# thorfdbg/libjpeg

Measured on AMD Instinct MI355X. Metric: decoded Mpixels/s, 8K 4:2:0 baseline (fused IDCT+upsample+YCbCr kernel, coefficients resident in HBM), higher is better.
Workload: dtype int32 (int16 coefficients in, u8 pixels out); 1 GPU; 64 x 7680x4320 4:2:0 Q85 DRI=8 baseline frames per GPU per step (BASELINE configs[2] frame shape, device-resident coefficient planes; 2 distinct pictures per rank repeated over the 64 frames: 6075 MiB in + 6075 MiB out per launch, far beyond the 256 MiB Infinity Cache); frames_per_gpu=64, kernel=fused420p_kernel, settle_launches=64, fast_arith=1, parallelism=image-sharded x1, no data-path collective

## Files before the change

### libjpeg_amd/csrc/kernels.hip

```cpp

#include <hip/hip_runtime.h>
#include <type_traits>
#include <stdint.h>
#include <stdlib.h>

#include "kernels.hpp"

namespace mij {

typedef unsigned u32x4 __attribute__((ext_vector_type(4)));
typedef unsigned u32x2 __attribute__((ext_vector_type(2)));
typedef u32x2 u32x2_any __attribute__((aligned(1)));
typedef u32x4 u32x4_any __attribute__((aligned(1)));
typedef int i32x4 __attribute__((ext_vector_type(4)));

template <bool FAST>
__device__ __forceinline__ int mulc(int a, int c)
{
  if (FAST) return __mul24(a, c);
  return (int)((unsigned)a * (unsigned)c);
}
__device__ __forceinline__ int addw(int a, int b) { return (int)((unsigned)a + (unsigned)b); }
__device__ __forceinline__ int subw(int a, int b) { return (int)((unsigned)a - (unsigned)b); }
__device__ __forceinline__ int shlw(int a, int n) { return (int)((unsigned)a << n); }
// ... 795 lines not shown
struct LdsPairHalf {
  short *cp;
  __device__ __forceinline__ LdsPairHalf(unsigned *cpair, int comp) : cp(reinterpret_cast<short *>(cpair) + comp) {}
  __device__ __forceinline__ void one(int at, int v) const { cp[2 * at] = (short)v; }
  __device__ __forceinline__ void row8(int at, const int *v) const
  {
    short *dst = cp + 2 * at;
#pragma unroll
    for (int x = 0; x < 8; x++) dst[2 * x] = (short)v[x];
  }
};
struct LdsPlane32 {
  int *cp;
  __device__ __forceinline__ LdsPlane32(int *plane) : cp(plane) {}
  __device__ __forceinline__ void one(int at, int v) const { cp[at] = v; }
  __device__ __forceinline__ void row8(int at, const int *v) const
  {
    i32x4 *dst = reinterpret_cast<i32x4 *>(cp + at);
    dst[0] = i32x4{v[0], v[1], v[2], v[3]};
    dst[1] = i32x4{v[4], v[5], v[6], v[7]};
  }
};

constexpr int F420P_MINW = 4;
constexpr int F420_FAST_MINW = 2;
constexpr int F420_12_MINW = 2;

struct NoAfterFetch { __device__ __forceinline__ void operator()() const {} };
template <bool FAST, bool QDEV = false, bool PK = false, class AfterFetch = NoAfterFetch>
__device__ __forceinline__ void f420_chroma_to_lds(const Fused420Args &a, const TileCtx &t, int (*cplane)[F420_CROWS * F420_CPITCH],
                                                   AfterFetch after_fetch = AfterFetch())
{
  const int16_t *__restrict__ coef = t.coef;
  u32x4 *stage = t.stage;
  const int lane = t.lane, wave = t.wave, tx = t.tx, ty = t.ty, frame = t.frame;
  const int comp = wave >> 1;
  const int16_t *__restrict__ plane = coef + (comp ? a.off_cr : a.off_cb);
  const int gx0 = tx * 8 - 1, gy0 = ty * 8 - 1;
  const int base = (wave & 1) * 64;
  const bool inside = gx0 >= 0 && gy0 >= 0 && gx0 + F420_CGRID <= a.bw_c && gy0 + F420_CGRID <= a.bh_c;
  u32x4 rows[8];
  const int idx0 = base + (lane >> 3);
  const char *pbase = reinterpret_cast<const char *>(plane) + (lane & 7) * 16;
  if (inside) {
    const unsigned off0 = (unsigned)((gy0 * a.bw_c + gx0) * 128), rowb = (unsigned)a.bw_c * 128u;
    fetch_blocks(rows, stage, lane, [&](int m) -> const u32x4 * {
      const unsigned i = (unsigned)min(idx0 + 8 * m, F420_CGRID * F420_CGRID - 1);
      const unsigned y = (i * 205u) >> 11, x = i - y * F420_CGRID;
      return reinterpret_cast<const u32x4 *>(pbase + (off0 + y * rowb + x * 128u));
    });
  } else {
    fetch_blocks(rows, stage, lane, [&](int m) -> const u32x4 * {
      const int i = min(idx0 + 8 * m, F420_CGRID * F420_CGRID - 1);
      const int y = (i * 205) >> 11, x = i - y * F420_CGRID;
      const int gx = min(max(gx0 + x, 0), a.bw_c - 1), gy = min(max(gy0 + y, 0), a.bh_c - 1);
      return reinterpret_cast<const u32x4 *>(pbase + (unsigned)((gy * a.bw_c + gx) * 128));
    });
  }
  after_fetch();
  if constexpr (!std::is_same<AfterFetch, NoAfterFetch>::value) __builtin_amdgcn_sched_barrier(0);
  const int idx = base + lane;
  const int cby = idx / F420_CGRID, cbx = idx - cby * F420_CGRID;
  const int gx = gx0 + cbx, gy = gy0 + cby;
  if (idx < F420_CGRID * F420_CGRID && gx >= 0 && gy >= 0 && gx < a.bw_c && gy < a.bh_c) {
    int v[64];
    const int *q = frame_deltas<QDEV>(a, frame, 1 + comp);
    if (FAST) dequant_idct_sparse<PK>(rows, q, v);
    else dequant_idct<false>(rows, q, v, 128 << 7);
    int *cp = cplane[comp];
#pragma unroll
    for (int r = 0; r < 8; r++) {
      const int pr = 8 * cby + r - 7;
      if (pr >= 0 && pr < F420_CROWS) {
        if (cbx == 0) {
          cp[pr * F420_CPITCH + 3] = v[r * 8 + 7];
        } else if (cbx == F420_CGRID - 1) {
          cp[pr * F420_CPITCH + 68] = v[r * 8 + 0];
        } else {
          i32x4 *dst = reinterpret_cast<i32x4 *>(cp + pr * F420_CPITCH + 8 * cbx - 4);
          dst[0] = i32x4{v[r * 8 + 0], v[r * 8 + 1], v[r * 8 + 2], v[r * 8 + 3]};
          dst[1] = i32x4{v[r * 8 + 4], v[r * 8 + 5], v[r * 8 + 6], v[r * 8 + 7]};
        }
      }
    }
  }
}

__device__ __forceinline__ void f420_chroma_edges(const Fused420Args &a, int (*cplane)[F420_CROWS * F420_CPITCH], int tid, int tx, int ty)
{
  const int last_col = a.cw - 1 - tx * 64;
  const int last_row = a.ch - 1 - ty * 64;
  const bool edge = (tx == 0) | (ty == 0) | (last_col < 64) | (last_row < 64);
  if (edge) {
    if (tid < 2 * F420_CROWS) {
      int *p = cplane[tid / F420_CROWS] + (tid % F420_CROWS) * F420_CPITCH;
      if (tx == 0) p[3] = p[4];
      if (last_col < 64) {
        const int v = p[last_col + 4];
        for (int pc = last_col + 5; pc <= 68; pc++) p[pc] = v;
      }
    }
    __syncthreads();
    if (tid < 2 * F420_CROWS) {
      int *p = cplane[tid / F420_CROWS] + 3 + (tid % F420_CROWS);
      if (ty == 0) p[0] = p[F420_CPITCH];
      if (last_row < 64) {
        const int v = p[(last_row + 1) * F420_CPITCH];
        for (int pr = last_row + 2; pr < F420_CROWS; pr++) p[pr * F420_CPITCH] = v;
      }
    }
    __syncthreads();
  }
}

constexpr int F422_CROWS = 128;
template <bool QDEV, bool PK16, class STORE>
__device__ __forceinline__ void f422_chroma_to_lds(const Fused420Args &a, const TileCtx &t, const STORE cp)
{
  const int lane = t.lane, wave = t.wave;
  const int comp = wave >> 1;
  const int16_t *__restrict__ plane = t.coef + (comp ? a.off_cr : a.off_cb);
  const int gx0 = t.tx * 8, gy0 = t.ty * 16 + (wave & 1) * 8;
  const char *pbase = reinterpret_cast<const char *>(plane) + (lane & 7) * 16;
  u32x4 rows[8];
  {
    const int xx = min(gx0 + (lane >> 3), a.bw_c - 1);
    fetch_blocks(rows, t.stage, lane, [&](int m) -> const u32x4 * {
      const int yy = min(gy0 + m, a.bh_c - 1);
      return reinterpret_cast<const u32x4 *>(pbase + (unsigned)((yy * a.bw_c + xx) * 128));
    });
    const int cbx = lane & 7, cby = lane >> 3;
    if (gx0 + cbx < a.bw_c && gy0 + cby < a.bh_c) {
      int v[64];
      dequant_idct_sparse<PK16>(rows, frame_deltas<QDEV>(a, t.frame, 1 + comp), v);
#pragma unroll
      for (int r = 0; r < 8; r++) cp.row8((8 * ((wave & 1) * 8 + cby) + r) * F420_CPITCH + 8 * cbx + 4, v + r * 8);
    }
  }
  {
    fetch_blocks16(rows, t.stage, lane, [&](int m) -> const u32x4 * {
      const int n = (lane >> 3) + 8 * m;
      const int xx = min(max((n & 1) ? gx0 + 8 : gx0 - 1, 0), a.bw_c - 1), yy = min(gy0 + (n >> 1), a.bh_c - 1);
      return reinterpret_cast<const u32x4 *>(pbase + (unsigned)((yy * a.bw_c + xx) * 128));
    });
    const int side = lane & 1, cby = lane >> 1, gx = side ? gx0 + 8 : gx0 - 1;
    if (lane < 16 && gx >= 0 && gx < a.bw_c && gy0 + cby < a.bh_c) {
      int col[8];
      dequant_idct_column(rows, frame_deltas<QDEV>(a, t.frame, 1 + comp), side == 0, col);
#pragma unroll
      for (int r = 0; r < 8; r++) cp.one((8 * ((wave & 1) * 8 + cby) + r) * F420_CPITCH + (side ? 68 : 3), col[r]);
    }
  }
}

template <int PLANES, class T>
__device__ __forceinline__ void f422_chroma_edges(const Fused420Args &a, T *lines, int tid, int tx)
{
  const int last_col = a.cw - 1 - tx * 64;
  if ((tx == 0) | (last_col < 64)) {
    if (tid < PLANES * F422_CROWS) {
      T *p = lines + tid * F420_CPITCH;
      if (tx == 0) p[3] = p[4];
      if (last_col < 64) {
        const T v = p[last_col + 4];
        for (int pc = last_col + 5; pc <= 68; pc++) p[pc] = v;
      }
    }
    __syncthreads();
  }
}

template <bool FAST, int MINW, bool QDEV, int P = 8, bool N12 = false, bool RAGGED = false>
__global__ __launch_bounds__(F420_THREADS, MINW) void fused420_kernel(Fused420Args a)
{
  static_assert(P == 8 || (P == 12 && FAST), "12-bit frames: FAST flavour only (the host checks the ranges)");
  static_assert(!RAGGED || (QDEV && P == 8), "ragged launches: 8 bit, per-frame tables");
  __shared__ __attribute__((aligned(16))) int cplane[2][F420_CROWS * F420_CPITCH];
  __shared__ __attribute__((aligned(16))) u32x4 stage_all[4][128];

  const TileCtx t = RAGGED ? tile_enter_ragged(a, stage_all) : tile_enter<P == 8 ? MIJ_TILE_ORDER : 1>(a, stage_all);
  if (t.padding) return;

  u32x4 yraw[8];
  auto luma_loads = [&]() { load_tile_blocks(yraw, t, t.coef + a.off_y, a.bw_y, a.bh_y); };
  constexpr bool PREFETCH = P == 8;
  if (PREFETCH) f420_chroma_to_lds<FAST, QDEV, !QDEV && P == 8>(a, t, cplane, luma_loads);
  else f420_chroma_to_lds<FAST, QDEV, !QDEV && P == 8>(a, t, cplane);
  __syncthreads();
  f420_chroma_edges(a, cplane, t.tid, t.tx, t.ty);

  u32x4 rows[8];
  if (!PREFETCH) luma_loads();
  transpose_blocks(rows, t.stage, t.lane, yraw);
  const BlockOut o = block_out<P == 12 ? 6 : 3>(a, t);
  if (o.outside) return;
  int yv[64];
  if (FAST) dequant_idct_sparse<!QDEV && P == 8, P == 8>(rows, frame_deltas<QDEV>(a, t.frame, 0), yv, 0, P == 8 ? LUMA_FOLD_R2 : 2048);
  else dequant_idct<false>(rows, frame_deltas<QDEV>(a, t.frame, 0), yv, 128 << 7);

  const int *cb_base = cplane[0] + (4 * o.by) * F420_CPITCH + 4 * o.bx;
  const int *cr_base = cplane[1] + (4 * o.by) * F420_CPITCH + 4 * o.bx;

  int cbT[6], cbC[6], cbB[6], crT[6], crC[6], crB[6];
  load6(cb_base, cbT); load6(cb_base + F420_CPITCH, cbC);
  load6(cr_base, crT); load6(cr_base + F420_CPITCH, crC);

#pragma unroll
  for (int m = 0; m < 4; m++) {
    load6(cb_base + (m + 2) * F420_CPITCH, cbB);
    load6(cr_base + (m + 2) * F420_CPITCH, crB);
#pragma unroll
    for (int half = 0; half < 2; half++) {
      const int l = 2 * m + half;
      int vb[6], vr[6];
#pragma unroll
      for (int j = 0; j < 6; j++) {
        const int rnd = ((j & 1) ^ half) ? 1 : 2;
        vb[j] = tap13(half ? cbB[j] : cbT[j], cbC[j], rnd);
        vr[j] = tap13(half ? crB[j] : crT[j], crC[j], rnd);
      }
      int ub[8], ur[8];
      hfilter8(vb, ub);
      hfilter8(vr, ur);
      if (l < o.nln) {
        if (FAST && P == 12) {
          int rr[8], gg[8], bb[8];
#pragma unroll
          for (int x = 0; x < 8; x++) colour12<N12>(yv[l * 8 + x], ub[x], ur[x], rr[x], gg[x], bb[x]);
          store_rgb12_line<F420_12_TEMPORAL>(o.out_frame + o.line_off(l, a), rr, gg, bb, o.fast_store, o.npx);
        } else if (FAST) {
          int rr[8], gg[8], bb[8];
#pragma unroll
          for (int x = 0; x < 8; x++) {
            const int yk = luma13(yv[l * 8 + x]);
            rr[x] = mad24(ur[x], L_CR_R, yk);
            gg[x] = mad24(ur[x], -L_CR_G, mad24(ub[x], -L_CB_G, yk));
            bb[x] = mad24(ub[x], L_CB_B, yk);
          }
          store_rgb8_line<STORE24_3X8>(o.out_frame, o.line_off(l, a), rr, gg, bb, o.fast_store, o.npx);
        } else {
          uint8_t *dst = o.out_frame + o.line_off(l, a);
          unsigned px[24];
#pragma unroll
          for (int x = 0; x < 8; x++) {
            int r, g, b;
            ycc_to_rgb<false>(yv[l * 8 + x], ub[x], ur[x], r, g, b);
            px[3 * x] = r; px[3 * x + 1] = g; px[3 * x + 2] = b;
          }
          if (o.fast_store) {
            unsigned w[6];
#pragma unroll
            for (int i = 0; i < 6; i++) w[i] = px[4 * i] | (px[4 * i + 1] << 8) | (px[4 * i + 2] << 16) | (px[4 * i + 3] << 24);
            store24_3x8(dst, w);
          } else {
#pragma unroll
            for (int x = 0; x < 8; x++)
              if (x < o.npx) {
                dst[3 * x] = (uint8_t)px[3 * x]; dst[3 * x + 1] = (uint8_t)px[3 * x + 1]; dst[3 * x + 2] = (uint8_t)px[3 * x + 2];
              }
          }
        }
      }
    }
#pragma unroll
    for (int j = 0; j < 6; j++) { cbT[j] = cbC[j]; cbC[j] = cbB[j]; crT[j] = crC[j]; crC[j] = crB[j]; }
  }
}

typedef short s16x2 __attribute__((ext_vector_type(2)));

__device__ __forceinline__ unsigned tap13_pk(unsigned a, unsigned b, short r)
{
  const s16x2 va = __builtin_bit_cast(s16x2, a), vb = __builtin_bit_cast(s16x2, b);
  const s16x2 t = (va + vb * (short)3 + r) >> (short)2;
  return __builtin_bit_cast(unsigned, t);
}
__device__ __forceinline__ unsigned centre3_pk(unsigned b, short r)
{
  unsigned d;
  asm("v_pk_mad_u16 %0, %1, 3, %2 op_sel_hi:[1,0,0]" : "=v"(d) : "v"(b), "n"(r));
  return d;
}
__device__ __forceinline__ unsigned tap_sum_pk(unsigned a, unsigned w)
{
  const s16x2 t = (__builtin_bit_cast(s16x2, a) + __builtin_bit_cast(s16x2, w)) >> (short)2;
  return __builtin_bit_cast(unsigned, t);
}

template <int MINW, bool QDEV, bool D2 = false, bool RAGGED = false>
__global__ __launch_bounds__(F420_THREADS, MINW) void fused420p_kernel(Fused420Args a)
{
  static_assert(!RAGGED || QDEV, "ragged launches: per-frame tables");
  __shared__ __attribute__((aligned(16))) unsigned cpair[F420_CROWS * F420_CPITCH];
  __shared__ __attribute__((aligned(16))) u32x4 stage_all[4][128];

  const TileCtx t = RAGGED ? tile_enter_ragged(a, stage_all) : tile_enter(a, stage_all);
  if (t.padding) return;
  const int tid = t.tid, lane = t.lane, wave = t.wave, frame = t.frame, tx = t.tx, ty = t.ty;
  u32x4 *stage = t.stage;
  const int16_t *__restrict__ coef = t.coef;
  u32x4 yraw[8];

  {
    const int comp = wave >> 1;
    const int16_t *__restrict__ plane = coef + (comp ? a.off_cr : a.off_cb);
    const int gx0 = tx * 8 - 1, gy0 = ty * 8 - 1;
    const int base = (wave & 1) * 64;
    const bool inside = gx0 >= 0 && gy0 >= 0 && gx0 + F420_CGRID <= a.bw_c && gy0 + F420_CGRID <= a.bh_c;
    u32x4 rows[8];
    const int idx0 = base + (lane >> 3);
    const char *pbase = reinterpret_cast<const char *>(plane) + (lane & 7) * 16;
    if (inside) {
      const unsigned off0 = (unsigned)((gy0 * a.bw_c + gx0) * 128), rowb = (unsigned)a.bw_c * 128u;
      fetch_blocks(rows, stage, lane, [&](int m) -> const u32x4 * {
        const unsigned i = (unsigned)min(idx0 + 8 * m, F420_CGRID * F420_CGRID - 1);
        const unsigned y = (i * 205u) >> 11, x = i - y * F420_CGRID;
        return reinterpret_cast<const u32x4 *>(pbase + (off0 + y * rowb + x * 128u));
      });
    } else {
      fetch_blocks(rows, stage, lane, [&](int m) -> const u32x4 * {
        const int i = min(idx0 + 8 * m, F420_CGRID * F420_CGRID - 1);
        const int y = (i * 205) >> 11, x = i - y * F420_CGRID;
        const int gx = min(max(gx0 + x, 0), a.bw_c - 1), gy = min(max(gy0 + y, 0), a.bh_c - 1);
        return reinterpret_cast<const u32x4 *>(pbase + (unsigned)((gy * a.bw_c + gx) * 128));
      });
    }
    const int idx = base + lane;
    const int cby = idx / F420_CGRID, cbx = idx - cby * F420_CGRID;
    const int gx = gx0 + cbx, gy = gy0 + cby;
    load_tile_blocks(yraw, t, coef + a.off_y, a.bw_y, a.bh_y);
    if (idx < F420_CGRID * F420_CGRID && gx >= 0 && gy >= 0 && gx < a.bw_c && gy < a.bh_c) {
      int v[64];
      dequant_idct_sparse<!QDEV, false, D2>(rows, frame_deltas<QDEV>(a, frame, 1 + comp), v);
      short *cp = reinterpret_cast<short *>(cpair) + comp;
#pragma unroll
      for (int r = 0; r < 8; r++) {
        const int pr = 8 * cby + r - 7;
        const int line = pr * F420_CPITCH;
        if (pr >= 0 && pr < F420_CROWS) {
          if (cbx == 0) {
            cp[2 * (line + 3)] = (short)v[r * 8 + 7];
          } else if (cbx == F420_CGRID - 1) {
            cp[2 * (line + 68)] = (short)v[r * 8 + 0];
          } else {
            short *dst = cp + 2 * (line + 8 * cbx - 4);
#pragma unroll
            for (int x = 0; x < 8; x++) dst[2 * x] = (short)v[r * 8 + x];
          }
        }
      }
    }
  }
  __syncthreads();

  {
    const int last_col = a.cw - 1 - tx * 64;
    const int last_row = a.ch - 1 - ty * 64;
    const bool edge = (tx == 0) | (ty == 0) | (last_col < 64) | (last_row < 64);
    if (edge) {
      if (tid < F420_CROWS) {
        unsigned *p = cpair + tid * F420_CPITCH;
        if (tx == 0) p[3] = p[4];
        if (last_col < 64) {
          const unsigned v = p[last_col + 4];
          for (int pc = last_col + 5; pc <= 68; pc++) p[pc] = v;
        }
      }
      __syncthreads();
      if (tid < F420_CROWS) {
        auto at = [&](int pr) -> unsigned & { return cpair[pr * F420_CPITCH + 3 + tid]; };
        if (ty == 0) at(0) = at(1);
        if (last_row < 64) {
          const unsigned v = at(last_row + 1);
          for (int pr = last_row + 2; pr < F420_CROWS; pr++) at(pr) = v;
        }
      }
      __syncthreads();
    }
  }

  u32x4 rows[8];
  transpose_blocks(rows, stage, lane, yraw);
  const BlockOut o = block_out<3>(a, t);
  if (o.outside) return;
  int yv[64];
  dequant_idct_sparse<!QDEV, true, D2>(rows, frame_deltas<QDEV>(a, frame, 0), yv, 0, LUMA_FOLD_R2);

  const int bx = o.bx, by = o.by, npx = o.npx, nln = o.nln;
  uint8_t *__restrict__ out_frame = o.out_frame;
  const unsigned out_off = o.out_off;
  const bool fast_store = o.fast_store;
  const unsigned *c_base = cpair + (4 * by) * F420_CPITCH + 4 * bx;

  const unsigned base_lo = (unsigned)(uintptr_t)out_frame;
  auto lines = [&](auto full_tag, auto shift_tag, auto staged_tag) {
    constexpr bool FULL = decltype(full_tag)::value, SHIFTED = decltype(shift_tag)::value, STAGED = decltype(staged_tag)::value;
    unsigned so0 = 0, so1 = 0;
    if (STAGED) {
      const unsigned wave_off = (unsigned)((ty * F420_TILE_BLOCKS + wave * 4) * 8) * (unsigned)a.row_stride + (unsigned)(tx * F420_TILE_BLOCKS * 8) * 3u;
      const unsigned c1 = 64u + (unsigned)lane;
      so0 = wave_off + ((unsigned)lane / 24u) * 8u * (unsigned)a.row_stride + ((unsigned)lane % 24u) * 16u;
      so1 = wave_off + (c1 / 24u) * 8u * (unsigned)a.row_stride + (c1 % 24u) * 16u;
    }
    unsigned cT[6], cC[6], cB[6];
    load6(c_base, cT);
    load6(c_base + F420_CPITCH, cC);
#pragma unroll
    for (int m = 0; m < 4; m++) {
      load6(c_base + (m + 2) * F420_CPITCH, cB);
      unsigned w1[6], w2[6];
#pragma unroll
      for (int j = 0; j < 6; j++) { w1[j] = centre3_pk(cC[j], 1); w2[j] = centre3_pk(cC[j], 2); }
#pragma unroll
      for (int half = 0; half < 2; half++) {
        const int l = 2 * m + half;
        unsigned v[6];
#pragma unroll
        for (int j = 0; j < 6; j++) v[j] = tap_sum_pk(half ? cB[j] : cT[j], ((j & 1) ^ half) ? w1[j] : w2[j]);
        unsigned u[8];
        u[7] = tap13_pk(v[5], v[4], 1);
        u[6] = tap13_pk(v[3], v[4], 2);
        u[5] = tap13_pk(v[4], v[3], 1);
        u[4] = tap13_pk(v[2], v[3], 2);
        u[3] = tap13_pk(v[3], v[2], 1);
        u[2] = tap13_pk(v[1], v[2], 2);
        u[1] = tap13_pk(u[2], v[1], 1);
        u[0] = tap13_pk(v[0], v[1], 2);
        if (FULL || l < nln) {
          int rr[8], gg[8], bb[8];
#pragma unroll
          for (int x = 0; x < 8; x++) {
            const int yk = luma13(yv[l * 8 + x]);
            rr[x] = mad16_hi(u[x], L_CR_R, yk);
            bb[x] = mad16_lo(u[x], L_CB_B, yk);
            gg[x] = dot2_16(u[x], -L_CB_G, -L_CR_G, yk);
          }
          if (FULL || fast_store) {
            unsigned w[6];
            rgb_shift17_sat_pack(rr, gg, bb, w);
            const unsigned off = out_off + (unsigned)l * (unsigned)a.row_stride;
            const int m = SHIFTED ? (int)__builtin_amdgcn_readfirstlane((base_lo + (unsigned)l * (unsigned)a.row_stride) & 3u) : 0;
            if (STAGED) {
              unsigned *sw = reinterpret_cast<unsigned *>(stage);
              u32x2 *pw = reinterpret_cast<u32x2 *>(sw + lane * 6);
              pw[0] = u32x2{w[0], w[1]}; pw[1] = u32x2{w[2], w[3]}; pw[2] = u32x2{w[4], w[5]};
              __builtin_amdgcn_wave_barrier();
              const u32x4 v0 = *reinterpret_cast<const u32x4 *>(sw + lane * 4);
              const u32x4 v1 = *reinterpret_cast<const u32x4 *>(sw + ((lane & 31) + 64) * 4);
              __builtin_amdgcn_wave_barrier();
              store16_nt(out_frame, so0 + (unsigned)l * (unsigned)a.row_stride, v0);
              if (lane < 32) store16_nt(out_frame, so1 + (unsigned)l * (unsigned)a.row_stride, v1);
            }
            else if (SHIFTED && m) store24_nt_shifted(out_frame, off, w, bx, m);
            else if (SHIFTED) store24_nt<false>(out_frame, off, w);
            else store24_nt(out_frame, off, w);
          } else {
            store_rgb8_partial(out_frame + (out_off + (unsigned)l * (unsigned)a.row_stride), rr, gg, bb, npx);
          }
        }
      }
#pragma unroll
      for (int j = 0; j < 6; j++) { cT[j] = cC[j]; cC[j] = cB[j]; }
    }
  };
  const bool whole = __builtin_amdgcn_ballot_w64(npx != 8 || nln != 8) == 0;
  if (whole && ((base_lo | (unsigned)a.row_stride) & 3u) && __builtin_amdgcn_ballot_w64(true) == ~0ull) lines(std::true_type{}, std::true_type{}, std::false_type{});
  else if (whole && __builtin_amdgcn_ballot_w64(true) == ~0ull) lines(std::true_type{}, std::false_type{}, std::true_type{});
  else if (whole) lines(std::true_type{}, std::false_type{}, std::false_type{});
  else lines(std::false_type{}, std::false_type{}, std::false_type{});
}

template <int MINW, bool QDEV, bool WIDE, bool RAGGED = false>
__global__ __launch_bounds__(F420_THREADS, MINW) void fused422_kernel(Fused420Args a)
{
  static_assert(!RAGGED || QDEV, "ragged launches: per-frame tables");
  __shared__ __attribute__((aligned(16))) unsigned cpair[F422_CROWS * F420_CPITCH];
  __shared__ __attribute__((aligned(16))) u32x4 stage_all[4][128];

  const TileCtx t = RAGGED ? tile_enter_ragged(a, stage_all) : tile_enter(a, stage_all);
  if (t.padding) return;

  f422_chroma_to_lds<QDEV, !QDEV>(a, t, LdsPairHalf(cpair, t.wave >> 1));
  __syncthreads();
  f422_chroma_edges<1>(a, cpair, t.tid, t.tx);

  u32x4 rows[8];
  fetch_tile_blocks(rows, t, t.coef + a.off_y, a.bw_y, a.bh_y);
  const BlockOut o = block_out<3>(a, t);
  if (o.outside) return;
  int yv[64];
  dequant_idct_sparse<!QDEV, true>(rows, frame_deltas<QDEV>(a, t.frame, 0), yv, 0, LUMA_FOLD_R2);

  const unsigned *c_base = cpair + (8 * o.by) * F420_CPITCH + 4 * o.bx;
#pragma unroll
  for (int l = 0; l < 8; l++) {
    {
      unsigned v[6];
      load6(c_base + l * F420_CPITCH, v);
      unsigned u[8];
      int ub[8], ur[8];
      if (WIDE) {
        int vb[6], vr[6];
#pragma unroll
        for (int j = 0; j < 6; j++) { vb[j] = (int)(short)(v[j] & 0xffffu); vr[j] = (int)v[j] >> 16; }
        hfilter8(vb, ub);
        hfilter8(vr, ur);
      } else {
        u[7] = tap13_pk(v[5], v[4], 1);
        u[6] = tap13_pk(v[3], v[4], 2);
        u[5] = tap13_pk(v[4], v[3], 1);
        u[4] = tap13_pk(v[2], v[3], 2);
        u[3] = tap13_pk(v[3], v[2], 1);
        u[2] = tap13_pk(v[1], v[2], 2);
        u[1] = tap13_pk(u[2], v[1], 1);
        u[0] = tap13_pk(v[0], v[1], 2);
      }
      if (l < o.nln) {
        int rr[8], gg[8], bb[8];
#pragma unroll
        for (int x = 0; x < 8; x++) {
          const int yk = luma13(yv[l * 8 + x]);
          if (WIDE) {
            rr[x] = mad24(ur[x], L_CR_R, yk);
            bb[x] = mad24(ub[x], L_CB_B, yk);
            gg[x] = mad24(ur[x], -L_CR_G, mad24(ub[x], -L_CB_G, yk));
          } else {
            rr[x] = mad16_hi(u[x], L_CR_R, yk);
            bb[x] = mad16_lo(u[x], L_CB_B, yk);
            gg[x] = dot2_16(u[x], -L_CB_G, -L_CR_G, yk);
          }
        }
        store_rgb8_line<STORE24_NT>(o.out_frame, o.line_off(l, a), rr, gg, bb, o.fast_store, o.npx);
      }
    }
  }
}

template <bool QDEV, bool N12>
__global__ __launch_bounds__(F420_THREADS, 2) void fused422_12_kernel(const Fused420Args a)
{
  __shared__ __attribute__((aligned(16))) int cplane[2][F422_CROWS * F420_CPITCH];
  __shared__ __attribute__((aligned(16))) u32x4 stage_all[4][128];

  const TileCtx t = tile_enter(a, stage_all);
  if (t.padding) return;

  f422_chroma_to_lds<QDEV, false>(a, t, LdsPlane32(cplane[t.wave >> 1]));
  __syncthreads();
  f422_chroma_edges<2>(a, cplane[0], t.tid, t.tx);

  u32x4 rows[8];
  fetch_tile_blocks(rows, t, t.coef + a.off_y, a.bw_y, a.bh_y);
  const BlockOut o = block_out<6>(a, t);
  if (o.outside) return;
  int yv[64];
  dequant_idct_sparse<false>(rows, frame_deltas<QDEV>(a, t.frame, 0), yv);

  const int *cb_base = cplane[0] + (8 * o.by) * F420_CPITCH + 4 * o.bx;
  const int *cr_base = cplane[1] + (8 * o.by) * F420_CPITCH + 4 * o.bx;
#pragma unroll
  for (int l = 0; l < 8; l++) {
    int vb[6], vr[6], ub[8], ur[8];
    load6(cb_base + l * F420_CPITCH, vb);
    load6(cr_base + l * F420_CPITCH, vr);
    hfilter8(vb, ub);
    hfilter8(vr, ur);
    if (l < o.nln) {
      int rr[8], gg[8], bb[8];
#pragma unroll
      for (int x = 0; x < 8; x++) colour12<N12>(yv[l * 8 + x], ub[x], ur[x], rr[x], gg[x], bb[x]);
      store_rgb12_line<F12_TEMPORAL>(o.out_frame + o.line_off(l, a), rr, gg, bb, o.fast_store, o.npx);
    }
  }
}

__device__ __forceinline__ int f8(int wa, int x, int wb, int y, int r);
__device__ __forceinline__ void hfilter4(const int (&s)[4], int (&o)[8])
{
  o[0] = f8(3, s[0], 5, s[1], 2); o[1] = f8(1, s[0], 7, s[1], 1); o[2] = f8(1, s[2], 7, s[1], 2); o[3] = f8(3, s[2], 5, s[1], 1);
  o[4] = f8(3, s[1], 5, s[2], 2); o[5] = f8(1, s[1], 7, s[2], 1); o[6] = f8(1, s[3], 7, s[2], 2); o[7] = f8(3, s[3], 5, s[2], 1);
}
constexpr int F411_CPITCH = 40;

template <int MINW, bool QDEV>
__global__ __launch_bounds__(F420_THREADS, MINW) void fused411_kernel(const Fused420Args a)
{
  __shared__ __attribute__((aligned(16))) unsigned cpair[F422_CROWS * F411_CPITCH];
  __shared__ __attribute__((aligned(16))) u32x4 stage_all[4][128];

  const TileCtx t = tile_enter(a, stage_all);
  if (t.padding) return;
  const int tid = t.tid, lane = t.lane, wave = t.wave, frame = t.frame, tx = t.tx, ty = t.ty;
  u32x4 *stage = t.stage;
  const int16_t *__restrict__ coef = t.coef;

  {
    const int comp = wave >> 1;
    const int16_t *__restrict__ plane = coef + (comp ? a.off_cr : a.off_cb);
    const int gx0 = tx * 4, gy0 = ty * 16;
    const char *pbase = reinterpret_cast<const char *>(plane) + (lane & 7) * 16;
    short *cp = reinterpret_cast<short *>(cpair) + comp;
    const int *qc = QDEV ? frame_deltas<QDEV>(a, frame, 1 + comp) : (comp ? a.q[2] : a.q[1]);
    u32x4 rows[8];
    if ((wave & 1) == 0) {
      fetch_blocks(rows, stage, lane, [&](int m) -> const u32x4 * {
        const int n = (lane >> 3) + 8 * m;
        const int xx = min(gx0 + (n & 3), a.bw_c - 1), yy = min(gy0 + (n >> 2), a.bh_c - 1);
        return reinterpret_cast<const u32x4 *>(pbase + (unsigned)((yy * a.bw_c + xx) * 128));
      });
      const int cbx = lane & 3, cby = lane >> 2;
      if (gx0 + cbx < a.bw_c && gy0 + cby < a.bh_c) {
        int v[64];
        dequant_idct_sparse<!QDEV>(rows, qc, v);
#pragma unroll
        for (int r = 0; r < 8; r++) {
          short *dst = cp + 2 * ((8 * cby + r) * F411_CPITCH + 8 * cbx + 4);
#pragma unroll
          for (int x = 0; x < 8; x++) dst[2 * x] = (short)v[r * 8 + x];
        }
      }
    } else {
      fetch_blocks(rows, stage, lane, [&](int m) -> const u32x4 * {
        const int n = min((lane >> 3) + 8 * m, 31);
        const int xx = min(max((n & 1) ? gx0 + 4 : gx0 - 1, 0), a.bw_c - 1), yy = min(gy0 + (n >> 1), a.bh_c - 1);
        return reinterpret_cast<const u32x4 *>(pbase + (unsigned)((yy * a.bw_c + xx) * 128));
      });
      const int side = lane & 1, cby = lane >> 1, gx = side ? gx0 + 4 : gx0 - 1;
      if (lane < 32 && gx >= 0 && gx < a.bw_c && gy0 + cby < a.bh_c) {
        int col[8];
        dequant_idct_column(rows, qc, side == 0, col);
#pragma unroll
        for (int r = 0; r < 8; r++) cp[2 * ((8 * cby + r) * F411_CPITCH + (side ? 36 : 3))] = (short)col[r];
      }
    }
  }
  __syncthreads();

  {
    const int last_col = a.cw - 1 - tx * 32;
    if ((tx == 0) | (last_col < 32)) {
      if (tid < F422_CROWS) {
        unsigned *p = cpair + tid * F411_CPITCH;
        if (tx == 0) p[3] = p[4];
        if (last_col < 32) {
          const unsigned v = p[last_col + 4];
          for (int pc = last_col + 5; pc <= 36; pc++) p[pc] = v;
        }
      }
      __syncthreads();
    }
  }

// ... 1969 lines not shown
```

Before: 923,900 Mpixels/s.

## Split chroma halo work into full-block IDCT waves and edge-only column/row IDCT waves

Chroma loading is reorganised. Two waves each decode the 64 interior chroma blocks of one component with a full IDCT. The other two waves decode only the halo: they run single-column IDCTs for the left and right neighbour blocks and corners, and single-row IDCTs for the above and below neighbours. This removes full 8x8 IDCTs on the 10x10 neighbour grid, where only one pixel row or column per block was used. The wave role assignment is also rotated by block index to balance work across SIMDs. The cost is more complex code with extra LDS transposes and scattered halo loads.

Measured after the change: 964,600 Mpixels/s, median of 6. 4.4% higher.

```diff
diff --git a/libjpeg_amd/csrc/kernels.hip b/libjpeg_amd/csrc/kernels.hip
--- a/libjpeg_amd/csrc/kernels.hip
+++ b/libjpeg_amd/csrc/kernels.hip
@@ -1121,52 +1121,105 @@
   u32x4 yraw[8];
 
   {
-    const int comp = wave >> 1;
+    const int role = (wave + (int)((blockIdx.x >> 3) + (blockIdx.x >> 8))) & 3;
+    const int comp = role & 1;
     const int16_t *__restrict__ plane = coef + (comp ? a.off_cr : a.off_cb);
-    const int gx0 = tx * 8 - 1, gy0 = ty * 8 - 1;
-    const int base = (wave & 1) * 64;
-    const bool inside = gx0 >= 0 && gy0 >= 0 && gx0 + F420_CGRID <= a.bw_c && gy0 + F420_CGRID <= a.bh_c;
-    u32x4 rows[8];
-    const int idx0 = base + (lane >> 3);
     const char *pbase = reinterpret_cast<const char *>(plane) + (lane & 7) * 16;
-    if (inside) {
-      const unsigned off0 = (unsigned)((gy0 * a.bw_c + gx0) * 128), rowb = (unsigned)a.bw_c * 128u;
+    const int *q = frame_deltas<QDEV>(a, frame, 1 + comp);
+    short *cp = reinterpret_cast<short *>(cpair) + comp;
+    const int gx0 = tx * 8, gy0 = ty * 8;
+    const int nb = lane >> 3;
+    if (role < 2) {
+      u32x4 rows[8];
+      const unsigned xoff = (unsigned)min(gx0 + nb, a.bw_c - 1) * 128u;
       fetch_blocks(rows, stage, lane, [&](int m) -> const u32x4 * {
-        const unsigned i = (unsigned)min(idx0 + 8 * m, F420_CGRID * F420_CGRID - 1);
-        const unsigned y = (i * 205u) >> 11, x = i - y * F420_CGRID;
-        return reinterpret_cast<const u32x4 *>(pbase + (off0 + y * rowb + x * 128u));
+        const int yy = min(gy0 + m, a.bh_c - 1);
+        return reinterpret_cast<const u32x4 *>(pbase + ((unsigned)(yy * a.bw_c) * 128u + xoff));
       });
+      load_tile_blocks(yraw, t, coef + a.off_y, a.bw_y, a.bh_y);
+      const int cbx = lane & 7, cby = lane >> 3;
+      if (gx0 + cbx < a.bw_c && gy0 + cby < a.bh_c) {
+        int at = (8 * cby + 1) * F420_CPITCH + 8 * cbx + 4;
+        if (QDEV) asm volatile("" : "+v"(at));
+        int v[64];
+        dequant_idct_sparse<!QDEV, false, D2>(rows, q, v);
+        short *dst = cp + 2 * at;
+#pragma unroll
+        for (int r = 0; r < 8; r++)
+#pragma unroll
+          for (int x = 0; x < 8; x++) dst[2 * (r * F420_CPITCH + x)] = (short)v[r * 8 + x];
+      }
     } else {
-      fetch_blocks(rows, stage, lane, [&](int m) -> const u32x4 * {
-        const int i = min(idx0 + 8 * m, F420_CGRID * F420_CGRID - 1);
-        const int y = (i * 205) >> 11, x = i - y * F420_CGRID;
-        const int gx = min(max(gx0 + x, 0), a.bw_c - 1), gy = min(max(gy0 + y, 0), a.bh_c - 1);
-        return reinterpret_cast<const u32x4 *>(pbase + (unsigned)((gy * a.bw_c + gx) * 128));
-      });
-    }
-    const int idx = base + lane;
-    const int cby = idx / F420_CGRID, cbx = idx - cby * F420_CGRID;
-    const int gx = gx0 + cbx, gy = gy0 + cby;
-    load_tile_blocks(yraw, t, coef + a.off_y, a.bw_y, a.bh_y);
-    if (idx < F420_CGRID * F420_CGRID && gx >= 0 && gy >= 0 && gx < a.bw_c && gy < a.bh_c) {
-      int v[64];
-      dequant_idct_sparse<!QDEV, false, D2>(rows, frame_deltas<QDEV>(a, frame, 1 + comp), v);
-      short *cp = reinterpret_cast<short *>(cpair) + comp;
-#pragma unroll
-      for (int r = 0; r < 8; r++) {
-        const int pr = 8 * cby + r - 7;
-        const int line = pr * F420_CPITCH;
-        if (pr >= 0 && pr < F420_CROWS) {
-          if (cbx == 0) {
-            cp[2 * (line + 3)] = (short)v[r * 8 + 7];
-          } else if (cbx == F420_CGRID - 1) {
-            cp[2 * (line + 68)] = (short)v[r * 8 + 0];
+      auto chunk = [&](int gx, int gy) -> u32x4 {
+        const int xx = min(max(gx, 0), a.bw_c - 1), yy = min(max(gy, 0), a.bh_c - 1);
+        return *reinterpret_cast<const u32x4 *>(pbase + (unsigned)((yy * a.bw_c + xx) * 128));
+      };
+      const int gxs = (nb & 1) ? gx0 + 8 : gx0 - 1;
+      const u32x4 side0 = chunk(gxs, gy0 + (nb >> 1)), side1 = chunk(gxs, gy0 + 4 + (nb >> 1));
+      const u32x4 corner = chunk(gxs, (nb & 2) ? gy0 + 8 : gy0 - 1);
+      const u32x4 above = chunk(gx0 + nb, gy0 - 1), below = chunk(gx0 + nb, gy0 + 8);
+      load_tile_blocks(yraw, t, coef + a.off_y, a.bw_y, a.bh_y);
+      {
+        u32x4 rows[8];
+        const int k = lane & 7;
+        stage[nb * 8 + (k ^ nb)] = side0;
+        stage[(nb + 8) * 8 + (k ^ nb)] = side1;
+        __builtin_amdgcn_wave_barrier();
+        if (lane < 16) {
+#pragma unroll
+          for (int r = 0; r < 8; r++) rows[r] = stage[lane * 8 + (r ^ (lane & 7))];
+        }
+        __builtin_amdgcn_wave_barrier();
+        stage[nb * 8 + (k ^ nb)] = corner;
+        __builtin_amdgcn_wave_barrier();
+        if (lane >= 16 && lane < 20) {
+#pragma unroll
+          for (int r = 0; r < 8; r++) rows[r] = stage[(lane - 16) * 8 + (r ^ (lane - 16))];
+        }
+        __builtin_amdgcn_wave_barrier();
+        const bool right = lane & 1, is_corner = lane >= 16, low = lane & 2;
+        const int gx = right ? gx0 + 8 : gx0 - 1, gy = is_corner ? (low ? gy0 + 8 : gy0 - 1) : gy0 + (lane >> 1);
+        if (lane < 20 && gx >= 0 && gx < a.bw_c && gy >= 0 && gy < a.bh_c) {
+          int col[8];
+          dequant_idct_column(rows, q, !right, col);
+          const int pc = right ? 68 : 3;
+          if (is_corner) {
+            cp[2 * ((low ? F420_CROWS - 1 : 0) * F420_CPITCH + pc)] = (short)(low ? col[0] : col[7]);
           } else {
-            short *dst = cp + 2 * (line + 8 * cbx - 4);
-#pragma unroll
-            for (int x = 0; x < 8; x++) dst[2 * x] = (short)v[r * 8 + x];
+            short *dst = cp + 2 * ((8 * (lane >> 1) + 1) * F420_CPITCH + pc);
+#pragma unroll
+            for (int r = 0; r < 8; r++) dst[2 * r * F420_CPITCH] = (short)col[r];
           }
         }
+      }
+      {
+        constexpr int W[8] = {512, FIX9(1.501321110) - FIX9(0.899976223) - FIX9(0.390180644) + FIX9(1.175875602), FIX9(0.541196100) + FIX9(0.765366865),
+                              FIX9(1.175875602), 512, FIX9(1.175875602) - FIX9(0.390180644), FIX9(0.541196100), FIX9(1.175875602) - FIX9(0.899976223)};
+        const int k = lane & 7;
+        typedef const __attribute__((address_space(4))) int kernarg_int;
+        int qrow[8];
+        if (QDEV) {
+          const int *qk = q + k * 8;
+#pragma unroll
+          for (int i = 0; i < 8; i++) qrow[i] = qk[i];
+        } else {
+          kernarg_int *qk = (kernarg_int *)__builtin_amdgcn_kernarg_segment_ptr() + (offsetof(Fused420Args, q) / sizeof(int) + (1 + comp) * QROW + k * 8);
+#pragma unroll
+          for (int i = 0; i < 8; i++) qrow[i] = qk[i];
+        }
+        const int weight = W[k];
+        int line[8];
+        short *dst = cp + 2 * (8 * nb + 4 + k);
+        const bool col_ok = gx0 + nb < a.bw_c;
+        auto mine = [&](const int (&l)[8]) {
+          const int a01 = (k & 1) ? l[1] : l[0], a23 = (k & 1) ? l[3] : l[2], a45 = (k & 1) ? l[5] : l[4], a67 = (k & 1) ? l[7] : l[6];
+          const int lo = (k & 2) ? a23 : a01, hi = (k & 2) ? a67 : a45;
+          return (short)((k & 4) ? hi : lo);
+        };
+        dequant_idct_line8(above, qrow, (k & 1) ? -weight : weight, line);
+        if (col_ok && gy0 > 0) dst[0] = mine(line);
+        dequant_idct_line8(below, qrow, weight, line);
+        if (col_ok && gy0 + 8 < a.bh_c) dst[2 * (F420_CROWS - 1) * F420_CPITCH] = mine(line);
       }
     }
   }
```
